# nextpyp/cet_pick

Hardware: AMD Instinct MI355X
Metric: subtomograms/sec (MoCo-3D train) + voxels/sec (heatmap+NMS) at 1/2/4/8 GPU (higher is better)
Workload: dtype f32; 1 GPU; moco_main.py moco3d_18: 3D encoder, synthetic 512x512x128 tomogram, 32^3 subtomo crops, batch 64 per GPU, r=1024, dim=128, m=0.999, T=0.1, SGD lr 1e-3; global_batch=64, parallelism=dp1, hipgraph=True

## Files before the change

### cet_pick_amd/_lib.py

```python
import ctypes
import os

import torch

_HERE = os.path.dirname(os.path.abspath(__file__))
LIB_PATH = os.environ.get("CETPICK_HIP_LIB") or os.path.join(_HERE, "libcetpick_hip.so")

_c = ctypes
_P, _I, _F, _Z, _D, _L = _c.c_void_p, _c.c_int, _c.c_float, _c.c_size_t, _c.c_double, _c.c_long

SIGNATURES = {
    "mi_abi_version": (_I, []),
    "mi_graph_node_counts": (_I, [_P, _P]),
    "mi_debug_stamp": (_I, [_P, _P]),
    "mi_linear_stats_fwd_f32": (_I, [_P] * 5 + [_I] * 3 + [_P]),
    "mi_debug_last_conv_kernel": (_c.c_char_p, []),
    "mi_linear_bn_fwd_f32": (_I, [_P] * 5 + [_I] * 3 + [_P, _P, _F, _F] + [_P] * 4 + [_I, _P]),
    "mi_conv3d_stem_stats_workspace_bytes": (_Z, [_I] * 5),
    "mi_conv3d_stem_stats_f32": (_I, [_P, _P, _P] + [_I] * 5 + [_P, _P, _Z, _P]),
    "mi_build_arch": (_c.c_char_p, []),
    "mi_sigmoid_clamp": (_I, [_P, _P, _Z, _P]),
    "mi_nms3d": (_I, [_P, _P, _I, _I, _I, _I, _I, _P]),
    "mi_decode_workspace_bytes": (_Z, [_I, _I, _I, _I]),
    "mi_decode_workspace_init": (_I, [_P, _Z, _P]),
# ... 123 lines not shown
    "mi_ce_label0": (_I, [_P, _P, _P, _P, _I, _I, _F, _P]),
    "mi_ce_label0_fwd": (_I, [_P, _P, _P, _P, _P, _I, _I, _P, _P]),
    "mi_ce_label0_bwd": (_I, [_P, _P, _P, _P, _I, _I, _P]),
    "mi_conv3d_s2_dgrad_usable": (_I, [_I, _I, _I, _I]),
    "mi_conv3d_s2_dgrad_workspace_bytes": (_Z, [_I, _I]),
    "mi_conv3d_s2_dgrad_f32": (_I, [_P] * 7 + [_I, _I, _I, _I, _P, _Z, _P]),
    "mi_conv3d_s2_fwd_usable": (_I, [_I, _I, _I, _I]),
    "mi_conv3d_s2_fwd_workspace_bytes": (_Z, [_I, _I]),
    "mi_conv3d_s2_fwd_f32": (_I, [_P] * 5 + [_I, _I, _I, _I, _P, _Z, _P]),
    "mi_conv3d_s2_prep": (_I, [_P] * 6 + [_I, _P]),
    "mi_conv3d_s2_fwd_img_f32": (_I, [_P] * 4 + [_I] * 4 + [_P]),
    "mi_conv3d_s2_dgrad_img_f32": (_I, [_P] * 6 + [_I] * 4 + [_P]),
    "mi_ema_update": (_I, [_P, _P, _F, _L, _P]),
    "mi_sgd_step": (_I, [_P, _P, _P, _F, _F, _F, _L, _P]),
    "mi_sgd_step2": (_I, [_P, _P, _P, _P, _F, _F, _F, _L, _P]),
    "mi_scalar_accumulate": (_I, [_P, _P, _P, _P, _P, _P]),
    "mi_queue_enqueue": (_I, [_P, _P, _P, _I, _I, _I, _P]),
    "mi_kmeans_image_bytes": (_Z, [_I, _I]),
    "mi_kmeans_workspace_bytes": (_Z, [_L, _I, _I]),
    "mi_kmeans_prep": (_I, [_P, _I, _I, _P, _P]),
    "mi_kmeans_xnorm": (_I, [_P, _L, _I, _P, _P]),
    "mi_kmeans_assign": (_I, [_P, _P, _P, _L, _I, _I, _P, _P, _P, _Z, _P]),
    "mi_kmeans_update": (_I, [_P, _P, _L, _I, _I, _P, _P, _P, _P, _P, _Z, _P]),
}

_lib = None


class HipExtensionError(RuntimeError):
    pass
# ... 80 lines not shown
```

### cet_pick_amd/csrc/conv_direct3.hip

```cpp
#include "common.h"
#include <type_traits>
#include <algorithm>

namespace {

using f32x16 = __attribute__((ext_vector_type(16))) float;
typedef __bf16 bf16x8 __attribute__((ext_vector_type(8)));
typedef unsigned u32x4 __attribute__((ext_vector_type(4)));

constexpr int C = 64;
constexpr int PLANE = 64;
constexpr int TZ = 2;
constexpr int PZ = TZ + 2;
constexpr int NV = PZ * PLANE;
constexpr int LEAD = 16;
constexpr int ZREC = 34;
constexpr int NREC = LEAD + NV + ZREC;
constexpr int ARR = NREC * 16;
constexpr int KS = C / 16;
constexpr int PL_BYTES = 2 * ARR;
constexpr int KS_BYTES = 3 * PL_BYTES;
constexpr int LDS_BYTES = KS * KS_BYTES;
constexpr int ZBASE = (LEAD + NV) * 16;
constexpr int WBLK = 1024;
constexpr int WSTEP = 2 * 3 * WBLK;
constexpr int NTAP = 27;
constexpr int NSTEP = KS * NTAP;
constexpr int WIMG_BYTES = NSTEP * WSTEP;
constexpr int RB = 6;
static_assert(NSTEP % RB == 0, "ring slots");
static_assert(LDS_BYTES <= 160 * 1024, "patch must fit the CU's LDS");
static_assert(((LEAD + NV) & 15) == 0, "zero region must start at a record = 0 (mod 16)");

struct Direct3Params {
    const float* a;
    const unsigned char* wimg;
    float* out;
    const float* res;
    const float* mask;
    int relu;
    int N, D;
    unsigned a_bytes;
};

__device__ __forceinline__ __amdgpu_buffer_rsrc_t rsrc_of(const void* base, unsigned bytes) {
    return __builtin_amdgcn_make_buffer_rsrc((void*)base, 0, (int)bytes, 0x00020000);
}

__device__ __forceinline__ void cut8(const float (&v)[8], u32x4 (&o)[3]) {
    unsigned u0[8], u1[8], u2[8];
#pragma unroll
    for (int t = 0; t < 8; ++t) {
        u0[t] = __float_as_uint(v[t]);
        const float r1 = v[t] - __uint_as_float(u0[t] & 0xffff0000u);
        u1[t] = __float_as_uint(r1);
        const float r2 = r1 - __uint_as_float(u1[t] & 0xffff0000u);
        u2[t] = __float_as_uint(r2);
    }
    constexpr unsigned HI2 = 0x07060302u;
#pragma unroll
    for (int d = 0; d < 4; ++d) {
        o[0][d] = __builtin_amdgcn_perm(u0[2 * d + 1], u0[2 * d], HI2);
        o[1][d] = __builtin_amdgcn_perm(u1[2 * d + 1], u1[2 * d], HI2);
        o[2][d] = __builtin_amdgcn_perm(u2[2 * d + 1], u2[2 * d], HI2);
    }
}

template <bool TWO, int CT = C>
__global__ __launch_bounds__(256, TWO ? 2 : 1) void direct3_kernel(Direct3Params p) {
    constexpr int KS = CT / 16, NSTEP = KS * NTAP;
    constexpr int NSLOT = TWO ? 2 : KS;
    static_assert(NSTEP % RB == 0, "ring slots");
    __shared__ __attribute__((aligned(16))) unsigned char patch[NSLOT * KS_BYTES];
    const int tid = threadIdx.x, lane = tid & 63, wave = tid >> 6;
    const int h = lane >> 5, l32 = lane & 31;
    const int tz = wave >> 1, cw = wave & 1;
    const int zb = blockIdx.x % (p.D / TZ), n = blockIdx.x / (p.D / TZ);
    const int z0 = zb * TZ;

    const int cb = blockIdx.y;
    const __amdgpu_buffer_rsrc_t wrs = rsrc_of(p.wimg, (CT / 64) * NSTEP * WSTEP);
// ... 398 lines not shown
    constexpr int KSn = CT / 16;
    const int lane = idx & 63, cw = (idx >> 6) & 1, rest = idx >> 7, ks = rest % KSn, tap = (rest / KSn) % NTAP, cb = rest / (KSn * NTAP);
    if (cb >= CT / 64) return;
    const int nn = cb * 64 + cw * 32 + (lane & 31), k0 = ks * 16 + 8 * (lane >> 5);
    float v[8];
    if (dgrad) {
        const float* src = w + ((long)(NTAP - 1 - tap) * CT + nn) * CT + k0;
        const float4 a = *reinterpret_cast<const float4*>(src), c = *reinterpret_cast<const float4*>(src + 4);
        v[0] = a.x; v[1] = a.y; v[2] = a.z; v[3] = a.w; v[4] = c.x; v[5] = c.y; v[6] = c.z; v[7] = c.w;
    } else {
#pragma unroll
        for (int e = 0; e < 8; ++e) v[e] = w[((long)tap * CT + k0 + e) * CT + nn];
    }
    u32x4 o[3];
    cut8(v, o);
    unsigned char* dst = img + (long)(((cb * KSn + ks) * NTAP + tap) * 2 + cw) * (3 * WBLK) + lane * 16;
#pragma unroll
    for (int pl = 0; pl < 3; ++pl) *reinterpret_cast<u32x4*>(dst + pl * WBLK) = o[pl];
}
__global__ __launch_bounds__(256) void direct3_prep_kernel(PrepBatch b) {
    const int fmt = b.wide[blockIdx.y], idx = blockIdx.x * 256 + threadIdx.x;
    if (fmt == 1) { if (blockIdx.x < PREP_BLOCKS_WIDE) direct3s_prep_body(b.w[blockIdx.y], b.img[blockIdx.y], b.dgrad[blockIdx.y], idx); }
    else if (fmt == 2) { if (blockIdx.x < PREP_BLOCKS_WIDE) direct3_prep_body<128>(b.w[blockIdx.y], b.img[blockIdx.y], b.dgrad[blockIdx.y], idx); }
    else if (fmt == 3) direct3s256_prep_body(b.w[blockIdx.y], b.img[blockIdx.y], b.dgrad[blockIdx.y], idx);
    else if (blockIdx.x < PREP_BLOCKS) direct3_prep_body<C>(b.w[blockIdx.y], b.img[blockIdx.y], b.dgrad[blockIdx.y], idx);
}


constexpr int WG_SPLITS = 28;
constexpr int WROW = 64;
constexpr int WHALF = (PLANE + 1) * WROW;
constexpr int WPL = 2 * WHALF;
constexpr int WOP = 3 * WPL;
// ... 477 lines not shown
    constexpr int NCB = CT / 32;
    const int lane = idx & 63, cb = (idx >> 6) % NCB, r1 = (idx >> 6) / NCB, ksx = r1 & 1, rest = r1 >> 1, tap = rest % NTAP, cc = rest / NTAP;
    if (cc >= NCB) return;
    const int nn = cb * 32 + (lane & 31), k0 = cc * 32 + ksx * 16 + 8 * (lane >> 5);
    float v[8];
    if (dgrad) {
        const float* src = w + ((long)(NTAP - 1 - tap) * CT + nn) * CT + k0;
        const float4 a = *reinterpret_cast<const float4*>(src), c = *reinterpret_cast<const float4*>(src + 4);
        v[0] = a.x; v[1] = a.y; v[2] = a.z; v[3] = a.w; v[4] = c.x; v[5] = c.y; v[6] = c.z; v[7] = c.w;
    } else {
#pragma unroll
        for (int e = 0; e < 8; ++e) v[e] = w[((long)tap * CT + k0 + e) * CT + nn];
    }
    u32x4 o[3];
    cut8(v, o);
    unsigned char* dst = img + (long)(((cc * NTAP + tap) * 2 + ksx) * NCB + cb) * (3 * WBLK) + lane * 16;
#pragma unroll
    for (int pl = 0; pl < 3; ++pl) *reinterpret_cast<u32x4*>(dst + pl * WBLK) = o[pl];
}
__device__ void direct3s_prep_body(const float* w, unsigned char* img, int dgrad, int idx) { direct3s_prep_body_t<CS>(w, img, dgrad, idx); }
__device__ void direct3s256_prep_body(const float* w, unsigned char* img, int dgrad, int idx) { direct3s_prep_body_t<256>(w, img, dgrad, idx); }

}

int mi_direct3_kind(int N, int Di, int Hi, int Wi, int Ci, int Co, int kd, int kh, int kw, int stride, int pd, int ph,
                    int pw, int dd, int dh, int dw) {
    const char* off = getenv("MI_CONV_NO_DIRECT");
    if (off && atoi(off) != 0) return 0;
    if (kd != 3 || kh != 3 || kw != 3 || stride != 1 || pd != 1 || ph != 1 || pw != 1 || dd != 1 || dh != 1 || dw != 1) return 0;
    if (N < 1 || 4l * N * Di * Hi * Wi * Ci >= 0x7fff0000l) return 0;
    if (Ci == C && Co == C && Hi == 8 && Wi == 8 && Di >= TZ && Di % TZ == 0) return 1;
    if (Ci == CS && Co == CS && Di == 4 && Hi == 4 && Wi == 4) return 2;
    if (Ci == 128 && Co == 128 && Hi == 8 && Wi == 8 && Di >= TZ && Di % TZ == 0 && (long)N * Di >= 128 && (long)N * (Di / TZ) <= 0x7fffffffl) return 3;
// ... 194 lines not shown
```

### cet_pick_amd/csrc/conv_s2.hip

```cpp
#include "common.h"
#include <algorithm>
#include <type_traits>

namespace {

using f32x16 = __attribute__((ext_vector_type(16))) float;
typedef __bf16 bf16x8 __attribute__((ext_vector_type(8)));
typedef unsigned u32x4 __attribute__((ext_vector_type(4)));

constexpr int S2_WBLK = 1024;

__device__ __forceinline__ __amdgpu_buffer_rsrc_t rsrc_s2(const void* base, unsigned bytes) {
    return __builtin_amdgcn_make_buffer_rsrc((void*)base, 0, (int)bytes, 0x00020000);
}

__device__ __forceinline__ void cut8s(const float (&v)[8], u32x4 (&o)[3]) {
    unsigned u0[8], u1[8], u2[8];
#pragma unroll
    for (int t = 0; t < 8; ++t) {
        u0[t] = __float_as_uint(v[t]);
        const float r1 = v[t] - __uint_as_float(u0[t] & 0xffff0000u);
        u1[t] = __float_as_uint(r1);
        u2[t] = __float_as_uint(r1 - __uint_as_float(u1[t] & 0xffff0000u));
    }
    constexpr unsigned HI2 = 0x07060302u;
#pragma unroll
    for (int d = 0; d < 4; ++d) {
        o[0][d] = __builtin_amdgcn_perm(u0[2 * d + 1], u0[2 * d], HI2);
        o[1][d] = __builtin_amdgcn_perm(u1[2 * d + 1], u1[2 * d], HI2);
        o[2][d] = __builtin_amdgcn_perm(u2[2 * d + 1], u2[2 * d], HI2);
    }
}

__host__ __device__ inline void s2_tap_of(int c, int j, int* tap, int* dz, int* dy, int* dx) {
    int d[3], t[3], bit = 0;
    for (int ax = 2; ax >= 0; --ax) {
        const int p = (c >> (2 - ax)) & 1;
        if (p) { d[ax] = (j >> bit) & 1; t[ax] = d[ax] ? 0 : 2; ++bit; }
        else { d[ax] = 0; t[ax] = 1; }
    }
    *tap = (t[0] * 3 + t[1]) * 3 + t[2];
    *dz = d[0]; *dy = d[1]; *dx = d[2];
}

struct S2DgradParams {
    const float* dh;
    const float* dout;
// ... 362 lines not shown
__global__ __launch_bounds__(256) void s2_prep_batch_kernel(S2PrepBatch b) {
    const S2PrepJob& jb = b.j[blockIdx.y];
    const long idx = (long)blockIdx.x * 256 + threadIdx.x;
    if (!jb.dgrad) {
        const int KS = jb.Ci / 16, CB = jb.Co / 32;
        const long per_e = (long)KS * CB * 64;
        if (idx >= 28 * per_e) return;
        const int lane = (int)(idx & 63), cbk = (int)((idx >> 6) % CB), ks = (int)((idx / (64 * CB)) % KS), e = (int)(idx / per_e);
        const int co = cbk * 32 + (lane & 31), ci0 = ks * 16 + 8 * (lane >> 5);
        const float* src = (e < 27 ? jb.w + (long)e * jb.Ci * jb.Co : jb.wds) + (long)ci0 * jb.Co + co;
        float v[8];
#pragma unroll
        for (int t = 0; t < 8; ++t) v[t] = src[(long)t * jb.Co];
        u32x4 o[3];
        cut8s(v, o);
        unsigned char* dst = jb.img + (((long)e * KS + ks) * CB + cbk) * (3 * S2_WBLK) + lane * 16;
#pragma unroll
        for (int pl = 0; pl < 3; ++pl) *reinterpret_cast<u32x4*>(dst + pl * S2_WBLK) = o[pl];
        return;
    }
    const int CR = jb.Co, CN = jb.Ci;
    const int KS = CR / 16, CB = CN / 32;
    const long per_tap = (long)KS * CB * 64;
    const long total = 27 * per_tap, total_ds = jb.wds ? per_tap : 0;
    if (idx >= total + total_ds) return;
    const bool ds = idx >= total;
    const long i = ds ? idx - total : idx;
    const int lane = (int)(i & 63), cbk = (int)((i >> 6) % CB), ks = (int)((i / (64 * CB)) % KS), slot = (int)(i / per_tap);
    const int ci = cbk * 32 + (lane & 31), co0 = ks * 16 + 8 * (lane >> 5);
    const float* src = ds ? jb.wds + (long)ci * CR + co0 : jb.w + ((long)b.slot_tap[slot] * CN + ci) * CR + co0;
    const float4 lo = *reinterpret_cast<const float4*>(src), hi = *reinterpret_cast<const float4*>(src + 4);
    const float v[8] = {lo.x, lo.y, lo.z, lo.w, hi.x, hi.y, hi.z, hi.w};
    u32x4 o[3];
    cut8s(v, o);
    unsigned char* dst = (ds ? jb.dsimg : jb.img) + (((long)(ds ? 0 : slot) * KS + ks) * CB + cbk) * (3 * S2_WBLK) + lane * 16;
#pragma unroll
    for (int pl = 0; pl < 3; ++pl) *reinterpret_cast<u32x4*>(dst + pl * S2_WBLK) = o[pl];
}

void s2_dgrad_tables(unsigned char order[8], unsigned char tap_off[8], unsigned char slot_tap[27]) {
    const int ord[8] = {7, 3, 5, 6, 1, 2, 4, 0};
    int slot = 0;
    for (int oi = 0; oi < 8; ++oi) {
        const int c = ord[oi];
        order[oi] = (unsigned char)c;
        tap_off[c] = (unsigned char)slot;
        const int nt = 1 << (((c >> 2) & 1) + ((c >> 1) & 1) + (c & 1));
        for (int j = 0; j < nt; ++j) {
            int tap, dz, dy, dxx;
            s2_tap_of(c, j, &tap, &dz, &dy, &dxx);
            slot_tap[slot++] = (unsigned char)tap;
        }
    }
}

}

extern "C" int mi_conv3d_s2_dgrad_usable(int N, int Gi, int Ci, int Co) {
    const char* off = getenv("MI_CONV_NO_DIRECT");
    if (off && atoi(off) != 0) return 0;
    const char* ar = getenv("MI_CONV_ARITH");
    if (ar && ar[0] == 'f') return 0;
    const char* no = getenv("MI_CONV_NO_S2");
    if (no && atoi(no) != 0) return 0;
    int G;
    return N >= 1 && s2_shape(Gi, Ci, Co, &G) && 4l * N * Gi * Gi * Gi * Ci < 0x7fff0000l ? 1 : 0;
}

extern "C" size_t mi_conv3d_s2_dgrad_workspace_bytes(int Ci, int Co) {
    return mi_align_up(s2_img_bytes(Ci, Co), 256) + mi_align_up(s2_dsimg_bytes(Ci, Co), 256);
// ... 131 lines not shown
```

### cet_pick_amd/csrc/train_ops.hip

```cpp
#include "common.h"
#include <algorithm>

namespace {

__device__ __forceinline__ float4 ld4(const float* p) { return *reinterpret_cast<const float4*>(p); }
__device__ __forceinline__ void st4(float* p, float4 v) { *reinterpret_cast<float4*>(p) = v; }

enum { CR_STATS = 0, CR_BNBWD = 1, CR_SUM = 2, CR_BNBWD_X = 3 };

struct PoolGeom { int N, Di, Hi, Wi, Do, Ho, Wo, k, s, pad; };

struct ColReduceParams {
    const float* a;
    const float* x;
    const float* y;
    const float* save;
    long M;
    int C, relu;
    double* partials;
    const float* gamma;
    const float* beta;
    double* sums_direct;
    float* f32_direct;
    int n_f32;
// ... 898 lines not shown
}
__global__ __launch_bounds__(256) void sgd_kernel(float* p, const float* g, const float* lr_dev,
                                                 float lr_host, float wd, float gs, long n) {
    const float lr = lr_dev ? *lr_dev : lr_host;
    long n4 = n >> 2;
    for (long i = (long)blockIdx.x * 256 + threadIdx.x; i < n4; i += (long)gridDim.x * 256) {
        float4 a = ld4(p + 4 * i), b = ld4(g + 4 * i);
        a.x -= lr * (gs * b.x + wd * a.x); a.y -= lr * (gs * b.y + wd * a.y);
        a.z -= lr * (gs * b.z + wd * a.z); a.w -= lr * (gs * b.w + wd * a.w);
        st4(p + 4 * i, a);
    }
    if (blockIdx.x == 0)
        for (long i = (n4 << 2) + threadIdx.x; i < n; i += 256) p[i] -= lr * (gs * g[i] + wd * p[i]);
}

__global__ void enqueue_kernel(float* queue, long long* ptr, const float* keys, int B, int C, int R) {
    const long long p0 = *ptr;
    for (int i = blockIdx.x * blockDim.x + threadIdx.x; i < B * C; i += gridDim.x * blockDim.x) {
        int b = i % B, c = i / B;
        long long col = p0 + b;
        if (col < R) queue[(long)c * R + col] = keys[(long)b * C + c];
    }
}
__global__ void advance_ptr_kernel(long long* ptr, int B, int R) { *ptr = (*ptr + B) % R; }
__global__ __launch_bounds__(1024) void enqueue_small_kernel(float* queue, long long* ptr, const float* keys, int B, int C, int R) {
    const long long p0 = *ptr;
    for (int i = threadIdx.x; i < B * C; i += 1024) {
        int b = i % B, c = i / B;
        long long col = p0 + b;
        if (col < R) queue[(long)c * R + col] = keys[(long)b * C + c];
// ... 436 lines not shown
    if (!k || !q || n <= 0 || ((uintptr_t)k & 15) || ((uintptr_t)q & 15)) return MI_E_ARG;
    hipLaunchKernelGGL(ema_kernel, dim3(ew_blocks(n / 4 + 1)), dim3(256), 0, (hipStream_t)stream, k, q, m, n);
    MI_RETURN_IF_LAUNCH_FAILED();
    return MI_OK;
}

extern "C" int mi_sgd_step(float* p, const float* g, const float* lr_dev, float lr, float weight_decay,
                           float grad_scale, long n, mi_stream_t stream) {
    if (!p || !g || n <= 0 || ((uintptr_t)p & 15) || ((uintptr_t)g & 15)) return MI_E_ARG;
    hipLaunchKernelGGL(sgd_kernel, dim3(ew_blocks(n / 4 + 1)), dim3(256), 0, (hipStream_t)stream, p, g, lr_dev, lr, weight_decay,
                       grad_scale, n);
    MI_RETURN_IF_LAUNCH_FAILED();
    return MI_OK;
}

__global__ __launch_bounds__(256) void sgd2_kernel(float* p, const float* g, const float* g2, const float* lr_dev, float lr_host, float wd,
                                                  float gs, long n) {
    const float lr = lr_dev ? *lr_dev : lr_host;
    long n4 = n >> 2;
    for (long i = (long)blockIdx.x * 256 + threadIdx.x; i < n4; i += (long)gridDim.x * 256) {
        float4 a = ld4(p + 4 * i), b = ld4(g + 4 * i), c = ld4(g2 + 4 * i);
        b.x += c.x; b.y += c.y; b.z += c.z; b.w += c.w;
        a.x -= lr * (gs * b.x + wd * a.x); a.y -= lr * (gs * b.y + wd * a.y);
        a.z -= lr * (gs * b.z + wd * a.z); a.w -= lr * (gs * b.w + wd * a.w);
        st4(p + 4 * i, a);
    }
    if (blockIdx.x == 0)
        for (long i = (n4 << 2) + threadIdx.x; i < n; i += 256) p[i] -= lr * (gs * (g[i] + g2[i]) + wd * p[i]);
}
extern "C" int mi_sgd_step2(float* p, const float* g, const float* g2, const float* lr_dev, float lr, float weight_decay,
// ... 36 lines not shown
```

### cet_pick_amd/hipops.py

```python
import os
import torch
import torch.nn as nn

from . import _lib as L


PROFILE = None
PROFILE_REPEAT = 8


def _prof_run(tag, flops, fn):
    fn()
    if PROFILE is not None:
        e0 = torch.cuda.Event(enable_timing=True)
        e1 = torch.cuda.Event(enable_timing=True)
        e0.record()
        for _ in range(PROFILE_REPEAT):
            fn()
        e1.record()
        PROFILE.append((tag, flops, e0, e1, PROFILE_REPEAT))


STAMPS = None

# ... 194 lines not shown
    n = len(items)
    if not n:
        return
    ws = (ctypes.c_void_p * n)(*[it[0].data_ptr() for it in items])
    imgs = (ctypes.c_void_p * n)(*[it[3].data_ptr() for it in items])
    dg = (ctypes.c_int * n)(*[it[2] for it in items])
    ch = (ctypes.c_int * n)(*[int(it[0].shape[0]) for it in items])
    cast = lambda a: ctypes.cast(a, ctypes.c_void_p)
    L.check(getattr(L.lib(), fn)(cast(ws), cast(imgs), cast(dg), cast(ch), n, L.stream()), fn)


class WeightImages:
    def __init__(self):
        self._groups = {}
        self._by_weight = {}

    def _family(self, group, fam):
        return self._groups.setdefault(group, {"s2": [], "direct": [], "p2d": []})[fam]

    @staticmethod
    def eligible(w, k, stride, pad):
        return (w.is_cuda and tuple(w.shape[:2]) in ((64, 64), (128, 128)) and _k3(k, True) == (3, 3, 3) and stride == 1
                and _p3(pad, True) == (1, 1, 1) and _phys_ok(w))

    def add(self, group, w, dgrad):
        nb = L.lib().mi_conv3d_direct_wimg_bytes(int(w.shape[0]))
        img = torch.empty(nb, dtype=torch.uint8, device=w.device)
        self._family(group, "direct").append((w, None, int(bool(dgrad)), img))
        self._by_weight[(w.data_ptr(), int(bool(dgrad)))] = img

# ... 38 lines not shown
        cast = lambda a: ctypes.cast(a, ctypes.c_void_p)
        L.check(L.lib().mi_conv3d_s2_prep(cast(ws), cast(wd), cast(imgs), cast(ci), cast(co), cast(dg), n, L.stream()),
                "mi_conv3d_s2_prep")

    def refresh(self, group):
        g = self._groups.get(group)
        if g is None:
            return
        self._refresh_s2(g["s2"])
        _prep_images("mi_conv3d_direct_prep", g["direct"])
        _prep_images("mi_conv2d_p2d_prep", g["p2d"])

    def refresh_all(self):
        for group in self._groups:
            self.refresh(group)

    def versions(self):
        return sum(it[0]._version + (it[1]._version if it[1] is not None else 0)
                   for g in self._groups.values() for items in g.values() for it in items)


def _arith_bf16x3():
    import os
    return not os.environ.get("MI_CONV_ARITH", "").startswith("f")


def _cached_image(w, dgrad, n, d, h, wd, k3, stride, p3):
    if ACTIVE_IMAGES is None or PROFILE is not None or k3 != (3, 3, 3) or stride != 1 or p3 != (1, 1, 1):
        return None
    if not _arith_bf16x3():
# ... 2045 lines not shown
```

### cet_pick_amd/models/moco.py

```python
import torch
import torch.nn as nn

from .. import hipops as H


class MoCo(nn.Module):
    def __init__(self, encoder_q, encoder_k, dim=32, r=1024, m=0.999, T=0.1):
        super().__init__()
        self.r, self.m, self.T = r, m, T
        self.encoder_q = encoder_q
        self.encoder_k = encoder_k
        for param_q, param_k in zip(self.encoder_q.parameters(), self.encoder_k.parameters()):
            param_k.data.copy_(param_q.data)
            param_k.requires_grad = False
        self.register_buffer("queue", torch.randn(dim, r))
        self.queue = nn.functional.normalize(self.queue, dim=0)
        self.register_buffer("queue_ptr", torch.zeros(1, dtype=torch.long))
        self._arena_q = self._arena_k = None

    def flatten_parameters(self):
        if self._arena_q is None or self._arena_q.flat.device != next(self.encoder_q.parameters()).device:
            self._arena_q = H.ParamArena(self.encoder_q)
            self._arena_k = H.ParamArena(self.encoder_k)
            assert self._arena_q.numel == self._arena_k.numel
        return self._arena_q, self._arena_k

    @torch.no_grad()
    def _momentum_update_key_encoder(self):
        if self._arena_q is not None:
            H.ema_update_(self._arena_k.flat, self._arena_q.flat, self.m)
            if self.weight_images is not None and H.ACTIVE_IMAGES is self.weight_images:
                self.weight_images.refresh("k")
            return
        for param_q, param_k in zip(self.encoder_q.parameters(), self.encoder_k.parameters()):
            n = param_q.numel()
            q = torch.as_strided(param_q.data, (n,), (1,))
            k = torch.as_strided(param_k.data, (n,), (1,))
            if n % 4 == 0 and k.data_ptr() % 16 == 0 and q.data_ptr() % 16 == 0:
                H.ema_update_(k, q, self.m)
            else:
                k.mul_(self.m).add_(q, alpha=1.0 - self.m)

    @torch.no_grad()
    def _dequeue_and_enqueue(self, keys):
# ... 167 lines not shown
```

### cet_pick_amd/trains/moco_engine.py

```python
import os

import torch

from .. import hipops as H
from .step_graph import StepGraph


class MocoStepEngine(StepGraph):
    def __init__(self, moco, lr, weight_decay=0.0, use_graph=False):
        self.moco = moco
        self.arena_q, self.arena_k = moco.flatten_parameters()
        super().__init__(moco, [self.arena_q, self.arena_k], lr, weight_decay, use_graph)
        dev = self.arena_q.flat.device
        self.logits = None
        self._one = torch.ones((), dtype=torch.float32, device=dev)
        self.loss = torch.zeros((), dtype=torch.float32, device=dev)
        self._loss_buf = self.loss
        self.loss_sum = torch.zeros((), dtype=torch.float32, device=dev)
        self._xchg = None
        self.buckets_sent = []
        if self.dist_on:
            self._setup_buckets()
        self.side_wgrads = dev.type == "cuda" and os.environ.get("CETPICK_SIDE_WGRADS", "1") != "0"
        self._wside = None
        self._wside_used = False
        self._wside_keep = []
        if self.side_wgrads:
            moco.encoder_q.grad_marker = self._on_marker
        self._images = self._build_weight_images()

    def _build_weight_images(self):
        if not self.arena_q.flat.is_cuda:
            return None
        imgs = H.WeightImages()
        for enc, group in ((self.moco.encoder_q, "q"), (self.moco.encoder_k, "k")):
            for m in enc.modules():
                if isinstance(m, H.HipConv3d) and H.WeightImages.eligible(m.weight, m.k, m.stride, m.pad):
                    imgs.add(group, m.weight, False)
                    if group == "q":
                        imgs.add(group, m.weight, True)
            for blk in enc.modules():
                ds = getattr(blk, "downsample", None)
                if ds is None or getattr(blk, "stride", 1) != 2 or not hasattr(blk, "conv1"):
                    continue
                w, wds = blk.conv1.weight, ds[0].weight
                co, ci = int(w.shape[0]), int(w.shape[1])
                if (co, ci) not in ((128, 64), (256, 128)) or not (H._phys_ok(w) and H._phys_ok(wds)):
                    continue
                imgs.add_s2(group, w, wds, False)
                if group == "q":
                    imgs.add_s2(group, w, wds, True)
        self.moco.weight_images = imgs
        return imgs

    def _setup_buckets(self):
        enc = self.moco.encoder_q
        first = {}
        for (name, _), off in zip(enc.named_parameters(), self.arena_q.offsets):
            first.setdefault(name.split(".")[0], off)
        end = self.arena_q.numel
        l1, l2, l3 = first["layer1"], first["layer2"], first["layer3"]
        self._bucket = {"layer3": (l3, end), "layer2": (l2, l3), "layer1": (l1, l2), "stem": (0, l1)}
        enc.grad_marker = self._on_marker

    def _reduce_bucket(self, tag):
        a, b = self._bucket[tag]
        H.flush_wgrad_reduces()
        if b > a and not self.arena_q.flat_grad.is_cuda:
            H.dist_all_reduce(self.arena_q.flat_grad[a:b])
            self.buckets_sent.append(tag)
        elif b > a:
            cur = torch.cuda.current_stream()
            if self._xchg is None:
                self._xchg = torch.cuda.Stream(device=self.arena_q.flat_grad.device)
            self._xchg.wait_stream(cur)
            if self._wside_used:
                self._xchg.wait_stream(self._wside)
            with torch.cuda.stream(self._xchg):
                H.dist_all_reduce(self.arena_q.flat_grad[a:b])
            self.buckets_sent.append(tag)

    def _on_marker(self, tag):
        if self.side_wgrads and tag in ("layer3", "layer2", "layer1"):
            self._issue_side_wgrads(enqueue=(tag == "layer3"))
        if self.dist_on:
            self._reduce_bucket(tag)

    def _issue_side_wgrads(self, enqueue=False):
        items = H.SIDE_WGRADS
        if not items:
            return
        cur = torch.cuda.current_stream()
        if H.PROFILE is not None:
            H.run_wgrad_jobs(items)
            H.flush_wgrad_reduces()
            if enqueue:
                self.moco.flush_enqueue()
            del items[:]
            return
        if self._wside is None:
            self._wside = torch.cuda.Stream(device=self.arena_q.flat_grad.device)
        self._wside.wait_stream(cur)
        with torch.cuda.stream(self._wside):
            H.run_wgrad_jobs(items)
            H.flush_wgrad_reduces()
            if enqueue:
                self._wside_keep.append(self.moco._pending_keys)
                self.moco.flush_enqueue()
        self._wside_keep.extend(items)
        del items[:]
        self._wside_used = True

    def step(self, im_q, im_k):
        return self._run({"q": im_q, "k": im_k})

    def step_eager(self, im_q, im_k):
        return self._run({"q": im_q, "k": im_k}, eager=True)

    def _step_eager(self, inputs):
        im_q, im_k = inputs["q"], inputs["k"]
        moco = self.moco
        self.buckets_sent = []
        self.arena_q.zero_grad()
        H.ACTIVE_IMAGES = self._images
        moco.defer_enqueue = True
        try:
            H.stamp("step:start")
            logits, labels = moco(im_q, im_k)
            self.logits = logits.detach()
            loss = H.cross_entropy_label0(logits, out=self._loss_buf)
            H.DEFERRED_WGRADS = [] if self.arena_q.flat_grad.is_cuda else None
            H.SIDE_WGRADS = [] if self.side_wgrads else None
            self._wside_used = False
            loss.backward(self._one)
            if H.SIDE_WGRADS:
                H.run_wgrad_jobs(H.SIDE_WGRADS)
            H.SIDE_WGRADS = None
# ... 1 lines not shown
                torch.cuda.current_stream().wait_stream(self._wside)
            del self._wside_keep[:]
            H.stamp("backward:end")
            H.flush_wgrad_reduces()
            moco.flush_enqueue()
        finally:
            H.DEFERRED_WGRADS = None
            H.SIDE_WGRADS = None
            H.ACTIVE_IMAGES = None
            moco.defer_enqueue = False
            moco._pending_keys = None
        if self.dist_on:
            self._reduce_bucket("stem")
            if self._xchg is not None:
                torch.cuda.current_stream().wait_stream(self._xchg)
        H.sgd_step_(self.arena_q.flat, self.arena_q.flat_grad, self.lr, self.weight_decay, self.lr_dev,
                    grad_scale=1.0 / self.world)
        if self._images is not None:
            self._images.refresh("q")
        self.loss_sum.add_(self.loss)
        H.stamp("step:end")
        return self.loss

    def take_loss_sum(self):
        v = float(self.loss_sum.item())
        self.loss_sum.zero_()
        return v
```

### include/cetpick_hip.h

```cpp
#ifndef CETPICK_HIP_H
#define CETPICK_HIP_H

#include <stddef.h>
#include <stdint.h>

#ifdef __cplusplus
extern "C" {
#endif

typedef void* mi_stream_t;

#define MI_OK 0
#define MI_E_ARG (-1)
#define MI_E_WORKSPACE (-2)
#define MI_E_UNSUPPORTED (-3)

int mi_abi_version(void);
int mi_graph_node_counts(void* graph, int* counts);
int mi_debug_stamp(void* slot, mi_stream_t stream);
const char* mi_debug_last_conv_kernel(void);
const char* mi_build_arch(void);


int mi_sigmoid_clamp(float* x, float* y, size_t n, mi_stream_t stream);
// ... 292 lines not shown
int mi_conv3d_s2_fwd_usable(int N, int Gi, int Ci, int Co);
size_t mi_conv3d_s2_fwd_workspace_bytes(int Ci, int Co);
int mi_conv3d_s2_fwd_f32(const float* x, const float* w, const float* w_ds, float* hmid, float* r, int N, int Gi, int Ci, int Co,
                         void* ws, size_t ws_bytes, mi_stream_t stream);

int mi_conv3d_s2_prep(const float* const* w, const float* const* w_ds, void* const* img, const int* ci, const int* co,
                      const int* dgrad, int n, mi_stream_t stream);
int mi_conv3d_s2_fwd_img_f32(const float* x, const void* img, float* hmid, float* r, int N, int Gi, int Ci, int Co,
                             mi_stream_t stream);
int mi_conv3d_s2_dgrad_img_f32(const float* dh, const float* dout, const void* img, float* dx, const float* res,
                               const float* mask, int N, int Gi, int Ci, int Co, mi_stream_t stream);

int mi_ema_update(float* k, const float* q, float m, long n, mi_stream_t stream);
int mi_sgd_step(float* p, const float* g, const float* lr_dev, float lr, float weight_decay, float grad_scale, long n,
                mi_stream_t stream);
int mi_sgd_step2(float* p, const float* g, const float* g2, const float* lr_dev, float lr, float weight_decay, float grad_scale, long n,
                 mi_stream_t stream);
int mi_scalar_accumulate(float* sums, const float* a, const float* b, const float* c, const float* d, mi_stream_t stream);
int mi_queue_enqueue(float* queue, int64_t* queue_ptr, const float* keys, int B, int C, int R,
                     mi_stream_t stream);

size_t mi_voxel_loss_workspace_bytes(long n);
int mi_pu_focal_loss_fwd(const float* pred, const float* gt, long n, double tau, double beta, double* sums,
                         float* loss, void* ws, size_t ws_bytes, mi_stream_t stream);
int mi_pu_focal_loss_bwd(const float* pred, const float* gt, long n, double tau, const double* sums,
                         const float* dloss, float* dpred, mi_stream_t stream);
int mi_focal_loss_fwd(const float* pred, const float* gt, long n, double* sums, float* loss, void* ws,
                      size_t ws_bytes, mi_stream_t stream);
int mi_focal_loss_bwd(const float* pred, const float* gt, long n, const double* sums, const float* dloss,
                      float* dpred, mi_stream_t stream);
// ... 27 lines not shown
```

Before: 42020 subtomograms/sec.

## Fuse SGD/EMA parameter updates with bf16-split weight image regeneration per bucket

Adds fused kernels that apply the SGD step or EMA update to the flat parameter arena and, in the same pass, rewrite the packed 3-plane bf16 forward and dgrad weight images for each conv weight. This replaces the separate update launch plus image refresh launches. The step boundary setting also lets per-layer SGD run early as gradient buckets complete, overlapping the optimizer with the rest of backward. The costs are an extra table-driven kernel path and more complex ordering between weight updates and weight-image consumers.

```diff
diff --git a/cet_pick_amd/_lib.py b/cet_pick_amd/_lib.py
--- a/cet_pick_amd/_lib.py
+++ b/cet_pick_amd/_lib.py
@@ -161,6 +161,8 @@
     "mi_ema_update": (_I, [_P, _P, _F, _L, _P]),
     "mi_sgd_step": (_I, [_P, _P, _P, _F, _F, _F, _L, _P]),
     "mi_sgd_step2": (_I, [_P, _P, _P, _P, _F, _F, _F, _L, _P]),
+    "mi_sgd_step_images": (_I, [_P, _P, _P, _F, _F, _F, _P, _I, _I, _I, _L, _P, _P, _P]),
+    "mi_ema_update_images": (_I, [_P, _P, _F, _P, _I, _I, _I, _L, _P]),
     "mi_scalar_accumulate": (_I, [_P, _P, _P, _P, _P, _P]),
     "mi_queue_enqueue": (_I, [_P, _P, _P, _I, _I, _I, _P]),
     "mi_kmeans_image_bytes": (_Z, [_I, _I]),
diff --git a/cet_pick_amd/csrc/conv_direct3.hip b/cet_pick_amd/csrc/conv_direct3.hip
--- a/cet_pick_amd/csrc/conv_direct3.hip
+++ b/cet_pick_amd/csrc/conv_direct3.hip
@@ -1,4 +1,5 @@
 #include "common.h"
+#include "wimg_layout.h"
 #include <type_traits>
 #include <algorithm>
 
@@ -22,7 +23,7 @@
 constexpr int KS_BYTES = 3 * PL_BYTES;
 constexpr int LDS_BYTES = KS * KS_BYTES;
 constexpr int ZBASE = (LEAD + NV) * 16;
-constexpr int WBLK = 1024;
+constexpr int WBLK = WIMG_BLK;
 constexpr int WSTEP = 2 * 3 * WBLK;
 constexpr int NTAP = 27;
 constexpr int NSTEP = KS * NTAP;
@@ -47,24 +48,7 @@
     return __builtin_amdgcn_make_buffer_rsrc((void*)base, 0, (int)bytes, 0x00020000);
 }
 
-__device__ __forceinline__ void cut8(const float (&v)[8], u32x4 (&o)[3]) {
-    unsigned u0[8], u1[8], u2[8];
-#pragma unroll
-    for (int t = 0; t < 8; ++t) {
-        u0[t] = __float_as_uint(v[t]);
-        const float r1 = v[t] - __uint_as_float(u0[t] & 0xffff0000u);
-        u1[t] = __float_as_uint(r1);
-        const float r2 = r1 - __uint_as_float(u1[t] & 0xffff0000u);
-        u2[t] = __float_as_uint(r2);
-    }
-    constexpr unsigned HI2 = 0x07060302u;
-#pragma unroll
-    for (int d = 0; d < 4; ++d) {
-        o[0][d] = __builtin_amdgcn_perm(u0[2 * d + 1], u0[2 * d], HI2);
-        o[1][d] = __builtin_amdgcn_perm(u1[2 * d + 1], u1[2 * d], HI2);
-        o[2][d] = __builtin_amdgcn_perm(u2[2 * d + 1], u2[2 * d], HI2);
-    }
-}
+__device__ __forceinline__ void cut8(const float (&v)[8], u32x4 (&o)[3]) { wimg_cut8(v, o); }
 
 template <bool TWO, int CT = C>
 __global__ __launch_bounds__(256, TWO ? 2 : 1) void direct3_kernel(Direct3Params p) {
@@ -493,9 +477,7 @@
     }
     u32x4 o[3];
     cut8(v, o);
-    unsigned char* dst = img + (long)(((cb * KSn + ks) * NTAP + tap) * 2 + cw) * (3 * WBLK) + lane * 16;
-#pragma unroll
-    for (int pl = 0; pl < 3; ++pl) *reinterpret_cast<u32x4*>(dst + pl * WBLK) = o[pl];
+    wimg_store(img + wimg_direct3_off<CT>(tap, k0, nn), o);
 }
 __global__ __launch_bounds__(256) void direct3_prep_kernel(PrepBatch b) {
     const int fmt = b.wide[blockIdx.y], idx = blockIdx.x * 256 + threadIdx.x;
@@ -1003,9 +985,7 @@
     }
     u32x4 o[3];
     cut8(v, o);
-    unsigned char* dst = img + (long)(((cc * NTAP + tap) * 2 + ksx) * NCB + cb) * (3 * WBLK) + lane * 16;
-#pragma unroll
-    for (int pl = 0; pl < 3; ++pl) *reinterpret_cast<u32x4*>(dst + pl * WBLK) = o[pl];
+    wimg_store(img + wimg_direct3s_off<CT>(tap, k0, nn), o);
 }
 __device__ void direct3s_prep_body(const float* w, unsigned char* img, int dgrad, int idx) { direct3s_prep_body_t<CS>(w, img, dgrad, idx); }
 __device__ void direct3s256_prep_body(const float* w, unsigned char* img, int dgrad, int idx) { direct3s_prep_body_t<256>(w, img, dgrad, idx); }
diff --git a/cet_pick_amd/csrc/conv_s2.hip b/cet_pick_amd/csrc/conv_s2.hip
--- a/cet_pick_amd/csrc/conv_s2.hip
+++ b/cet_pick_amd/csrc/conv_s2.hip
@@ -1,4 +1,5 @@
 #include "common.h"
+#include "wimg_layout.h"
 #include <algorithm>
 #include <type_traits>
 
@@ -8,29 +9,13 @@
 typedef __bf16 bf16x8 __attribute__((ext_vector_type(8)));
 typedef unsigned u32x4 __attribute__((ext_vector_type(4)));
 
-constexpr int S2_WBLK = 1024;
+constexpr int S2_WBLK = WIMG_BLK;
 
 __device__ __forceinline__ __amdgpu_buffer_rsrc_t rsrc_s2(const void* base, unsigned bytes) {
     return __builtin_amdgcn_make_buffer_rsrc((void*)base, 0, (int)bytes, 0x00020000);
 }
 
-__device__ __forceinline__ void cut8s(const float (&v)[8], u32x4 (&o)[3]) {
-    unsigned u0[8], u1[8], u2[8];
-#pragma unroll
-    for (int t = 0; t < 8; ++t) {
-        u0[t] = __float_as_uint(v[t]);
-        const float r1 = v[t] - __uint_as_float(u0[t] & 0xffff0000u);
-        u1[t] = __float_as_uint(r1);
-        u2[t] = __float_as_uint(r1 - __uint_as_float(u1[t] & 0xffff0000u));
-    }
-    constexpr unsigned HI2 = 0x07060302u;
-#pragma unroll
-    for (int d = 0; d < 4; ++d) {
-        o[0][d] = __builtin_amdgcn_perm(u0[2 * d + 1], u0[2 * d], HI2);
-        o[1][d] = __builtin_amdgcn_perm(u1[2 * d + 1], u1[2 * d], HI2);
-        o[2][d] = __builtin_amdgcn_perm(u2[2 * d + 1], u2[2 * d], HI2);
-    }
-}
+__device__ __forceinline__ void cut8s(const float (&v)[8], u32x4 (&o)[3]) { wimg_cut8(v, o); }
 
 __host__ __device__ inline void s2_tap_of(int c, int j, int* tap, int* dz, int* dy, int* dx) {
     int d[3], t[3], bit = 0;
@@ -423,9 +408,7 @@
         for (int t = 0; t < 8; ++t) v[t] = src[(long)t * jb.Co];
         u32x4 o[3];
         cut8s(v, o);
-        unsigned char* dst = jb.img + (((long)e * KS + ks) * CB + cbk) * (3 * S2_WBLK) + lane * 16;
-#pragma unroll
-        for (int pl = 0; pl < 3; ++pl) *reinterpret_cast<u32x4*>(dst + pl * S2_WBLK) = o[pl];
+        wimg_store(jb.img + wimg_s2_off(e, ci0, co, KS, CB), o);
         return;
     }
     const int CR = jb.Co, CN = jb.Ci;
@@ -442,9 +425,7 @@
     const float v[8] = {lo.x, lo.y, lo.z, lo.w, hi.x, hi.y, hi.z, hi.w};
     u32x4 o[3];
     cut8s(v, o);
-    unsigned char* dst = (ds ? jb.dsimg : jb.img) + (((long)(ds ? 0 : slot) * KS + ks) * CB + cbk) * (3 * S2_WBLK) + lane * 16;
-#pragma unroll
-    for (int pl = 0; pl < 3; ++pl) *reinterpret_cast<u32x4*>(dst + pl * S2_WBLK) = o[pl];
+    wimg_store((ds ? jb.dsimg : jb.img) + wimg_s2_off(ds ? 0 : slot, co0, ci, KS, CB), o);
 }
 
 void s2_dgrad_tables(unsigned char order[8], unsigned char tap_off[8], unsigned char slot_tap[27]) {
@@ -463,6 +444,12 @@
     }
 }
 
+}
+
+void mi_s2_dgrad_tap_slots(unsigned char tap_slot[27]) {
+    unsigned char order[8], tap_off[8], slot_tap[27];
+    s2_dgrad_tables(order, tap_off, slot_tap);
+    for (int s = 0; s < 27; ++s) tap_slot[slot_tap[s]] = (unsigned char)s;
 }
 
 extern "C" int mi_conv3d_s2_dgrad_usable(int N, int Gi, int Ci, int Co) {
diff --git a/cet_pick_amd/csrc/train_ops.hip b/cet_pick_amd/csrc/train_ops.hip
--- a/cet_pick_amd/csrc/train_ops.hip
+++ b/cet_pick_amd/csrc/train_ops.hip
@@ -1,5 +1,7 @@
 #include "common.h"
+#include "wimg_layout.h"
 #include <algorithm>
+#include <type_traits>
 
 namespace {
 
@@ -936,6 +938,122 @@
         for (long i = (n4 << 2) + threadIdx.x; i < n; i += 256) p[i] -= lr * (gs * g[i] + wd * p[i]);
 }
 
+struct WimgItem {
+    long long off;
+    unsigned char* fwd;
+    unsigned char* dg;
+    int ntap, ci, co;
+    int fam;
+    int e0;
+    int blk0;
+};
+struct WimgSeg { long long start, n; };
+struct WimgTable {
+    const WimgItem* items; const WimgSeg* segs;
+    int n_items, n_segs, ew_blocks, img_blocks;
+    unsigned char tap_slot[27];
+};
+
+struct SgdUpdate {
+    float lr, gs, wd;
+    __device__ __forceinline__ float operator()(float p, float g) const { float a = p; a -= lr * (gs * g + wd * a); return a; }
+};
+struct EmaUpdate {
+    float m, om;
+    __device__ __forceinline__ float operator()(float k, float q) const { return k * m + q * om; }
+};
+
+template <class U>
+__device__ __forceinline__ void wimg_tile(const U& upd, float* p, const float* g, const WimgItem& it, const unsigned char* tap_slot,
+                                          int tile) {
+    const int cot_n = it.co >> 3, cit_n = it.ci >> 3;
+    const int cot = tile % cot_n, r1 = tile / cot_n, cit = r1 % cit_n, tap = r1 / cit_n;
+    if (tap >= it.ntap) return;
+    const int ci0 = cit * 8, co0 = cot * 8;
+    const long base = it.off + ((long)tap * it.ci + ci0) * it.co + co0;
+    const int dtap = it.fam == 2 ? (it.e0 ? 27 : tap_slot[tap]) : 26 - tap;
+    float nv[8][8];
+#pragma unroll
+    for (int r = 0; r < 8; ++r) {
+        const long o = base + (long)r * it.co;
+        const float4 a0 = ld4(p + o), a1 = ld4(p + o + 4), b0 = ld4(g + o), b1 = ld4(g + o + 4);
+        const float a[8] = {a0.x, a0.y, a0.z, a0.w, a1.x, a1.y, a1.z, a1.w}, b[8] = {b0.x, b0.y, b0.z, b0.w, b1.x, b1.y, b1.z, b1.w};
+#pragma unroll
+        for (int c = 0; c < 8; ++c) nv[r][c] = upd(a[c], b[c]);
+        st4(p + o, make_float4(nv[r][0], nv[r][1], nv[r][2], nv[r][3]));
+        st4(p + o + 4, make_float4(nv[r][4], nv[r][5], nv[r][6], nv[r][7]));
+    }
+    wimg_u32x4 o3[3];
+    if (it.dg) {
+#pragma unroll
+        for (int r = 0; r < 8; ++r) {
+            wimg_cut8(nv[r], o3);
+            const long d = it.fam == 0 ? wimg_direct3_off<64>(dtap, co0, ci0 + r) : it.fam == 1 ? wimg_direct3s_off<128>(dtap, co0, ci0 + r)
+                         : wimg_s2_off(dtap, co0, ci0 + r, it.co >> 4, it.ci >> 5);
+            wimg_store(it.dg + d, o3);
+        }
+    }
+    if (it.fwd) {
+#pragma unroll
+        for (int c = 0; c < 8; ++c) {
+            const float v[8] = {nv[0][c], nv[1][c], nv[2][c], nv[3][c], nv[4][c], nv[5][c], nv[6][c], nv[7][c]};
+            wimg_cut8(v, o3);
+            const long d = it.fam == 0 ? wimg_direct3_off<64>(tap, ci0, co0 + c) : it.fam == 1 ? wimg_direct3s_off<128>(tap, ci0, co0 + c)
+                         : wimg_s2_off(it.e0 + tap, ci0, co0 + c, it.ci >> 4, it.co >> 5);
+            wimg_store(it.fwd + d, o3);
+        }
+    }
+}
+
+template <class U>
+__global__ __launch_bounds__(256) void wimg_update_kernel(float* p, const float* g, const float* lr_dev, U upd, WimgTable t,
+                                                         float* acc, const float* acc_src) {
+    if (lr_dev) {
+        if constexpr (std::is_same<U, SgdUpdate>::value) upd.lr = *lr_dev;
+    }
+    if ((int)blockIdx.x >= t.ew_blocks) {
+        const int b = (int)blockIdx.x - t.ew_blocks;
+        int i = 0;
+        while (i + 1 < t.n_items && t.items[i + 1].blk0 <= b) ++i;
+        const WimgItem it = t.items[i];
+        wimg_tile(upd, p, g, it, t.tap_slot, (b - it.blk0) * 256 + (int)threadIdx.x);
+        return;
+    }
+    if (acc && blockIdx.x == 0 && threadIdx.x == 0) *acc += *acc_src;
+    const long stride = (long)t.ew_blocks * 256;
+    for (int s = 0; s < t.n_segs; ++s) {
+        const WimgSeg sg = t.segs[s];
+        float* ps = p + sg.start;
+        const float* gs = g + sg.start;
+        const long n4 = sg.n >> 2;
+        long i = (long)blockIdx.x * 256 + threadIdx.x;
+        for (; i + stride < n4; i += 2 * stride) {
+            float4 a = ld4(ps + 4 * i), b = ld4(gs + 4 * i), c = ld4(ps + 4 * (i + stride)), d = ld4(gs + 4 * (i + stride));
+            a.x = upd(a.x, b.x); a.y = upd(a.y, b.y); a.z = upd(a.z, b.z); a.w = upd(a.w, b.w);
+            c.x = upd(c.x, d.x); c.y = upd(c.y, d.y); c.z = upd(c.z, d.z); c.w = upd(c.w, d.w);
+            st4(ps + 4 * i, a); st4(ps + 4 * (i + stride), c);
+        }
+        if (i < n4) {
+            float4 a = ld4(ps + 4 * i), b = ld4(gs + 4 * i);
+            a.x = upd(a.x, b.x); a.y = upd(a.y, b.y); a.z = upd(a.z, b.z); a.w = upd(a.w, b.w);
+            st4(ps + 4 * i, a);
+        }
+        if (blockIdx.x == 0)
+            for (long j = (n4 << 2) + threadIdx.x; j < sg.n; j += 256) ps[j] = upd(ps[j], gs[j]);
+    }
+}
+
+int ew_blocks(long n);
+int wimg_table_of(const void* table, int n_items, int n_segs, int img_blocks, long seg_elems, WimgTable* t) {
+    if (!table || n_items < 0 || n_segs < 0 || n_items + n_segs == 0 || img_blocks < 0 || ((uintptr_t)table & 15)) return MI_E_ARG;
+    t->items = (const WimgItem*)table;
+    t->segs = (const WimgSeg*)((const unsigned char*)table + sizeof(WimgItem) * (size_t)n_items);
+    t->n_items = n_items; t->n_segs = n_segs; t->img_blocks = n_items ? img_blocks : 0;
+    t->ew_blocks = n_segs ? ew_blocks(seg_elems / 4 + 1) : 1;
+    mi_s2_dgrad_tap_slots(t->tap_slot);
+    return MI_OK;
+}
+
 __global__ void enqueue_kernel(float* queue, long long* ptr, const float* keys, int B, int C, int R) {
     const long long p0 = *ptr;
     for (int i = blockIdx.x * blockDim.x + threadIdx.x; i < B * C; i += gridDim.x * blockDim.x) {
@@ -1402,6 +1520,35 @@
     return MI_OK;
 }
 
+static int wimg_check_launch(const WimgTable& t) { return (long)t.ew_blocks + t.img_blocks > 0x7fffffffl ? MI_E_ARG : MI_OK; }
+
+extern "C" int mi_sgd_step_images(float* p, const float* g, const float* lr_dev, float lr, float weight_decay, float grad_scale,
+                                  const void* table, int n_items, int n_segs, int img_blocks, long seg_elems, float* acc,
+                                  const float* acc_src, mi_stream_t stream) {
+    if (!p || !g || ((uintptr_t)p & 15) || ((uintptr_t)g & 15) || ((acc == nullptr) != (acc_src == nullptr))) return MI_E_ARG;
+    WimgTable t;
+    int rc = wimg_table_of(table, n_items, n_segs, img_blocks, seg_elems, &t);
+    if (rc || (rc = wimg_check_launch(t))) return rc;
+    SgdUpdate u = {lr, grad_scale, weight_decay};
+    hipLaunchKernelGGL(wimg_update_kernel<SgdUpdate>, dim3((unsigned)(t.ew_blocks + t.img_blocks)), dim3(256), 0, (hipStream_t)stream, p, g,
+                       lr_dev, u, t, acc, acc_src);
+    MI_RETURN_IF_LAUNCH_FAILED();
+    return MI_OK;
+}
+
+extern "C" int mi_ema_update_images(float* k, const float* q, float m, const void* table, int n_items, int n_segs, int img_blocks,
+                                    long seg_elems, mi_stream_t stream) {
+    if (!k || !q || ((uintptr_t)k & 15) || ((uintptr_t)q & 15)) return MI_E_ARG;
+    WimgTable t;
+    int rc = wimg_table_of(table, n_items, n_segs, img_blocks, seg_elems, &t);
+    if (rc || (rc = wimg_check_launch(t))) return rc;
+    EmaUpdate u = {m, 1.0f - m};
+    hipLaunchKernelGGL(wimg_update_kernel<EmaUpdate>, dim3((unsigned)(t.ew_blocks + t.img_blocks)), dim3(256), 0, (hipStream_t)stream, k, q,
+                       (const float*)nullptr, u, t, (float*)nullptr, (const float*)nullptr);
+    MI_RETURN_IF_LAUNCH_FAILED();
+    return MI_OK;
+}
+
 __global__ __launch_bounds__(256) void sgd2_kernel(float* p, const float* g, const float* g2, const float* lr_dev, float lr_host, float wd,
                                                   float gs, long n) {
     const float lr = lr_dev ? *lr_dev : lr_host;
diff --git a/cet_pick_amd/csrc/wimg_layout.h b/cet_pick_amd/csrc/wimg_layout.h
--- /dev/null
+++ b/cet_pick_amd/csrc/wimg_layout.h
@@ -0,0 +1,48 @@
+#pragma once
+#include <hip/hip_runtime.h>
+
+typedef unsigned wimg_u32x4 __attribute__((ext_vector_type(4)));
+
+constexpr int WIMG_BLK = 1024;
+
+__device__ __forceinline__ void wimg_cut8(const float (&v)[8], wimg_u32x4 (&o)[3]) {
+    unsigned u0[8], u1[8], u2[8];
+#pragma unroll
+    for (int t = 0; t < 8; ++t) {
+        u0[t] = __float_as_uint(v[t]);
+        const float r1 = v[t] - __uint_as_float(u0[t] & 0xffff0000u);
+        u1[t] = __float_as_uint(r1);
+        const float r2 = r1 - __uint_as_float(u1[t] & 0xffff0000u);
+        u2[t] = __float_as_uint(r2);
+    }
+    constexpr unsigned HI2 = 0x07060302u;
+#pragma unroll
+    for (int d = 0; d < 4; ++d) {
+        o[0][d] = __builtin_amdgcn_perm(u0[2 * d + 1], u0[2 * d], HI2);
+        o[1][d] = __builtin_amdgcn_perm(u1[2 * d + 1], u1[2 * d], HI2);
+        o[2][d] = __builtin_amdgcn_perm(u2[2 * d + 1], u2[2 * d], HI2);
+    }
+}
+
+__device__ __forceinline__ int wimg_lane(int k0, int n) { return (n & 31) + 32 * ((k0 >> 3) & 1); }
+
+template <int CT>
+__device__ __forceinline__ long wimg_direct3_off(int tap, int k0, int n) {
+    const int cb = n >> 6, cw = (n >> 5) & 1, ks = k0 >> 4;
+    return (long)(((cb * (CT / 16) + ks) * 27 + tap) * 2 + cw) * (3 * WIMG_BLK) + wimg_lane(k0, n) * 16;
+}
+template <int CT>
+__device__ __forceinline__ long wimg_direct3s_off(int tap, int k0, int n) {
+    const int cb = n >> 5, cc = k0 >> 5, ksx = (k0 >> 4) & 1;
+    return (long)(((cc * 27 + tap) * 2 + ksx) * (CT / 32) + cb) * (3 * WIMG_BLK) + wimg_lane(k0, n) * 16;
+}
+__device__ __forceinline__ long wimg_s2_off(int entry, int k0, int n, int KS, int CB) {
+    return (((long)entry * KS + (k0 >> 4)) * CB + (n >> 5)) * (3 * WIMG_BLK) + wimg_lane(k0, n) * 16;
+}
+
+__device__ __forceinline__ void wimg_store(unsigned char* dst, const wimg_u32x4 (&o)[3]) {
+#pragma unroll
+    for (int pl = 0; pl < 3; ++pl) *reinterpret_cast<wimg_u32x4*>(dst + pl * WIMG_BLK) = o[pl];
+}
+
+void mi_s2_dgrad_tap_slots(unsigned char tap_slot[27]);
diff --git a/cet_pick_amd/hipops.py b/cet_pick_amd/hipops.py
--- a/cet_pick_amd/hipops.py
+++ b/cet_pick_amd/hipops.py
@@ -232,6 +232,8 @@
     def __init__(self):
         self._groups = {}
         self._by_weight = {}
+        self._tables = {}
+        self.fused = False
 
     def _family(self, group, fam):
         return self._groups.setdefault(group, {"s2": [], "direct": [], "p2d": []})[fam]
@@ -300,6 +302,70 @@
     def refresh_all(self):
         for group in self._groups:
             self.refresh(group)
+
+    def _fused_table(self, group, flat, rng):
+        import struct
+        a, b = (0, flat.numel()) if rng is None else (int(rng[0]), int(rng[1]))
+        key = (group, flat.data_ptr(), a, b)
+        tab = self._tables.get(key)
+        if tab is not None:
+            return tab
+        g = self._groups.get(group) or {"s2": [], "direct": [], "p2d": []}
+        if g["p2d"]:
+            raise L.HipExtensionError("the optimiser kernels do not write conv_p2d images: refresh() them")
+        ent = {}
+        def note(w, fam, e0, dgrad, img):
+            if w.dtype != torch.float32 or not _phys_ok(w) or (w.data_ptr() - flat.data_ptr()) % 16:
+                raise L.HipExtensionError("imaged weight is not a kernel-layout fp32 view of the arena")
+            off = (w.data_ptr() - flat.data_ptr()) // 4
+            e = ent.setdefault(off, [w, fam, e0, 0, 0])
+            if e[1] != fam or e[2] != e0 or e[3 + dgrad]:
+                raise L.HipExtensionError("two images of one kind for one weight")
+            e[3 + dgrad] = img.data_ptr()
+        for w, _, dgrad, img in g["direct"]:
+            note(w, 0 if int(w.shape[0]) == 64 else 1, 0, dgrad, img)
+        for w, wds, dgrad, img in g["s2"]:
+            note(w, 2, 0, dgrad, img)
+            if wds is not None:
+                note(wds, 2, 27, dgrad, img)
+        items, segs, pos, blk = [], [], a, 0
+        for off in sorted(ent):
+            w, fam, e0, fwd, dg = ent[off]
+            co, ci = int(w.shape[0]), int(w.shape[1])
+            ntap = w.numel() // (co * ci)
+            if off + w.numel() <= a or off >= b:
+                continue
+            if off < pos or off + w.numel() > b or ci % 32 or co % 32:
+                raise L.HipExtensionError("imaged weight straddles the range (%d, %d) or overlaps another" % (a, b))
+            if off > pos:
+                segs.append((pos, off - pos))
+            items.append(struct.pack("<qQQiiiiii", off, fwd, dg, ntap, ci, co, fam, e0, blk))
+            blk += (ntap * (ci // 8) * (co // 8) + 255) // 256
+            pos = off + w.numel()
+        if b > pos:
+            segs.append((pos, b - pos))
+        if a % 4 or any(s % 4 for s, _ in segs):
+            raise L.HipExtensionError("arena range (%d, %d) is not 16-byte aligned" % (a, b))
+        raw = b"".join(items) + b"".join(struct.pack("<qq", s, n) for s, n in segs)
+        dev = torch.frombuffer(bytearray(raw), dtype=torch.uint8).to(flat.device) if raw else None
+        tab = (dev, len(items), len(segs), blk, sum(n for _, n in segs))
+        self._tables[key] = tab
+        return tab
+
+    def refresh_fused(self, group, flat, src, rng=None, ema=None, sgd=None, acc=None):
+        tab, n_items, n_segs, blocks, seg_elems = self._fused_table(group, flat, rng)
+        if tab is None:
+            return
+        _bump_weight_epoch()
+        lib = L.lib()
+        if ema is not None:
+            L.check(lib.mi_ema_update_images(L.ptr(flat), L.ptr(src), float(ema), L.ptr(tab), n_items, n_segs, blocks, seg_elems,
+                                             L.stream()), "mi_ema_update_images")
+            return
+        lr, wd, lr_dev, gs = sgd
+        acc_p, acc_s = (L.ptr(acc[0]), L.ptr(acc[1])) if acc is not None else (None, None)
+        L.check(lib.mi_sgd_step_images(L.ptr(flat), L.ptr(src), L.ptr(lr_dev), float(lr), float(wd), float(gs), L.ptr(tab), n_items, n_segs,
+                                       blocks, seg_elems, acc_p, acc_s, L.stream()), "mi_sgd_step_images")
 
     def versions(self):
         return sum(it[0]._version + (it[1]._version if it[1] is not None else 0)
diff --git a/cet_pick_amd/models/moco.py b/cet_pick_amd/models/moco.py
--- a/cet_pick_amd/models/moco.py
+++ b/cet_pick_amd/models/moco.py
@@ -28,6 +28,9 @@
     @torch.no_grad()
     def _momentum_update_key_encoder(self):
         if self._arena_q is not None:
+            if self.weight_images is not None and H.ACTIVE_IMAGES is self.weight_images and self.weight_images.fused:
+                self.weight_images.refresh_fused("k", self._arena_k.flat, self._arena_q.flat, ema=self.m)
+                return
             H.ema_update_(self._arena_k.flat, self._arena_q.flat, self.m)
             if self.weight_images is not None and H.ACTIVE_IMAGES is self.weight_images:
                 self.weight_images.refresh("k")
diff --git a/cet_pick_amd/trains/moco_engine.py b/cet_pick_amd/trains/moco_engine.py
--- a/cet_pick_amd/trains/moco_engine.py
+++ b/cet_pick_amd/trains/moco_engine.py
@@ -28,6 +28,15 @@
         if self.side_wgrads:
             moco.encoder_q.grad_marker = self._on_marker
         self._images = self._build_weight_images()
+        self.boundary = int(os.environ.get("CETPICK_STEP_BOUNDARY", "2")) if self._images is not None else 0
+        self._sgd_done = []
+        if self._images is not None:
+            self._images.fused = self.boundary >= 1
+        if self.boundary >= 2 and not self.dist_on:
+            if all(hasattr(moco.encoder_q, t) for t in ("layer1", "layer2", "layer3")):
+                self._setup_ranges()
+            else:
+                self.boundary = 1
 
     def _build_weight_images(self):
         if not self.arena_q.flat.is_cuda:
@@ -54,6 +63,10 @@
         return imgs
 
     def _setup_buckets(self):
+        self._setup_ranges()
+        self.moco.encoder_q.grad_marker = self._on_marker
+
+    def _setup_ranges(self):
         enc = self.moco.encoder_q
         first = {}
         for (name, _), off in zip(enc.named_parameters(), self.arena_q.offsets):
@@ -61,9 +74,8 @@
         end = self.arena_q.numel
         l1, l2, l3 = first["layer1"], first["layer2"], first["layer3"]
         self._bucket = {"layer3": (l3, end), "layer2": (l2, l3), "layer1": (l1, l2), "stem": (0, l1)}
-        enc.grad_marker = self._on_marker
-
-    def _reduce_bucket(self, tag):
+
+    def _reduce_bucket(self, tag, sgd=False):
         a, b = self._bucket[tag]
         H.flush_wgrad_reduces()
         if b > a and not self.arena_q.flat_grad.is_cuda:
@@ -78,15 +90,28 @@
                 self._xchg.wait_stream(self._wside)
             with torch.cuda.stream(self._xchg):
                 H.dist_all_reduce(self.arena_q.flat_grad[a:b])
+                if sgd:
+                    self._sgd_bucket_early(tag)
             self.buckets_sent.append(tag)
 
+    def _sgd_range(self, rng, acc=None):
+        self._images.refresh_fused("q", self.arena_q.flat, self.arena_q.flat_grad, rng=rng,
+                                   sgd=(self.lr, self.weight_decay, self.lr_dev, 1.0 / self.world), acc=acc)
+
+    def _sgd_bucket_early(self, tag):
+        a, b = self._bucket[tag]
+        if b > a:
+            self._sgd_range((a, b))
+            self._sgd_done.append(tag)
+
     def _on_marker(self, tag):
+        early = self.boundary >= 2 and H.PROFILE is None and tag in ("layer3", "layer2", "layer1")
         if self.side_wgrads and tag in ("layer3", "layer2", "layer1"):
-            self._issue_side_wgrads(enqueue=(tag == "layer3"))
+            self._issue_side_wgrads(enqueue=(tag == "layer3"), sgd_tag=tag if early and not self.dist_on else None)
         if self.dist_on:
-            self._reduce_bucket(tag)
-
-    def _issue_side_wgrads(self, enqueue=False):
+            self._reduce_bucket(tag, sgd=early and self.arena_q.flat_grad.is_cuda)
+
+    def _issue_side_wgrads(self, enqueue=False, sgd_tag=None):
         items = H.SIDE_WGRADS
         if not items:
             return
@@ -107,6 +132,8 @@
             if enqueue:
                 self._wside_keep.append(self.moco._pending_keys)
                 self.moco.flush_enqueue()
+            if sgd_tag is not None:
+                self._sgd_bucket_early(sgd_tag)
         self._wside_keep.extend(items)
         del items[:]
         self._wside_used = True
@@ -121,6 +148,7 @@
         im_q, im_k = inputs["q"], inputs["k"]
         moco = self.moco
         self.buckets_sent = []
+        self._sgd_done = []
         self.arena_q.zero_grad()
         H.ACTIVE_IMAGES = self._images
         moco.defer_enqueue = True
@@ -152,6 +180,19 @@
             self._reduce_bucket("stem")
             if self._xchg is not None:
                 torch.cuda.current_stream().wait_stream(self._xchg)
+        if self.boundary >= 1:
+            acc = (self.loss_sum, self.loss)
+            if not self._sgd_done:
+                self._sgd_range(None, acc)
+            else:
+                left = [t for t in ("layer3", "layer2", "layer1", "stem") if t not in self._sgd_done
+                        and self._bucket[t][1] > self._bucket[t][0]]
+                for i, t in enumerate(left):
+                    self._sgd_range(self._bucket[t], acc if i == len(left) - 1 else None)
+                if not left:
+                    self.loss_sum.add_(self.loss)
+            H.stamp("step:end")
+            return self.loss
         H.sgd_step_(self.arena_q.flat, self.arena_q.flat_grad, self.lr, self.weight_decay, self.lr_dev,
                     grad_scale=1.0 / self.world)
         if self._images is not None:
diff --git a/include/cetpick_hip.h b/include/cetpick_hip.h
--- a/include/cetpick_hip.h
+++ b/include/cetpick_hip.h
@@ -330,6 +330,10 @@
 int mi_ema_update(float* k, const float* q, float m, long n, mi_stream_t stream);
 int mi_sgd_step(float* p, const float* g, const float* lr_dev, float lr, float weight_decay, float grad_scale, long n,
                 mi_stream_t stream);
+int mi_sgd_step_images(float* p, const float* g, const float* lr_dev, float lr, float weight_decay, float grad_scale, const void* table,
+                       int n_items, int n_segs, int img_blocks, long seg_elems, float* acc, const float* acc_src, mi_stream_t stream);
+int mi_ema_update_images(float* k, const float* q, float m, const void* table, int n_items, int n_segs, int img_blocks, long seg_elems,
+                         mi_stream_t stream);
 int mi_sgd_step2(float* p, const float* g, const float* g2, const float* lr_dev, float lr, float weight_decay, float grad_scale, long n,
                  mi_stream_t stream);
 int mi_scalar_accumulate(float* sums, const float* a, const float* b, const float* c, const float* d, mi_stream_t stream);
```

Result: slower. 40850 subtomograms/sec (-2.8%).
